# cristiano-nicolau/sudoku_solver_distributed

Measured on AMD Instinct MI355X. Metric: puzzles solved/sec (node), 1M hard 9x9 batch @1/2/4/8 GPU; single-puzzle p50 ms, higher is better.
Workload: dtype u8; 1 GPU; hard 17-clue 9x9 batch, 1048576 boards per step over all GPUs; global_batch=1048576, parallelism=shard1, steps_per_launch=32, inflight_per_gpu=2

## Files before the change

### sudoku_solver_distributed_amd/build.py

```python
from __future__ import annotations

import os
import subprocess
import sys

_HERE = os.path.dirname(os.path.abspath(__file__))
ROOT = os.path.dirname(_HERE)
_SCHED = os.environ.get("SDK_PLANE_SCHED", "iterative-ilp")


_LLVM_EXTRA = os.environ.get("SDK_PLANE_LLVM", "").split()


def sources(sched: str = _SCHED):
    extra = [f for o in _LLVM_EXTRA for f in ("-mllvm", o)]
    return (("sudoku_kernels.hip", []),
            ("plane_kernels.hip", ([] if sched == "default" else ["-mllvm", f"-amdgpu-sched-strategy={sched}"]) + extra),
            ("count_kernels.hip", ["-mllvm", "-amdgpu-sched-strategy=iterative-minreg"]),
            ("canon_kernels.hip", []),
            ("rate_kernels.hip", []),
            ("cand_kernels.hip", ["-mllvm", "-amdgpu-sched-strategy=iterative-minreg"]),
            ("min_kernels.hip", ["-mllvm", "-amdgpu-sched-strategy=iterative-minreg"]),
            ("sample_kernels.hip", ["-mllvm", "-amdgpu-sched-strategy=iterative-minreg"]),
            ("uniq_kernels.hip", ["-mllvm", "-amdgpu-sched-strategy=iterative-minreg"]),
            ("exact_kernels.hip", ["-mllvm", "-amdgpu-sched-strategy=iterative-minreg"]),
            ("enum_kernels.hip", ["-mllvm", "-amdgpu-sched-strategy=iterative-minreg"]),
            ("backdoor_kernels.hip", []),
            ("ua_kernels.hip", []),
            ("hit_kernels.hip", []))


SRCS = sources()
VARIANTS = {
    "default": ((), _SCHED),
    "stamps": (("SDK_PLANE_STAMPS=1",), _SCHED),
    "waves5": (("SDK_PLANE_WAVES_PER_EU=5",), _SCHED),
    "waves6": (("SDK_PLANE_WAVES_PER_EU=6",), _SCHED),
    "nopinacc": (("SDK_PLANE_PIN_ACC=0",), _SCHED),
    "sched-default": ((), "default"),
    "sched-minreg": ((), "iterative-minreg"),
    "sched-maxocc": ((), "iterative-maxocc"),
    "sched-max-ilp": ((), "max-ilp"),
}
OUT = os.path.join(_HERE, "libsudoku_hip.so")
ARCH = os.environ.get("SDK_OFFLOAD_ARCH", "gfx950")


def hipcc() -> str:
    for cand in (os.environ.get("HIPCC"), "/opt/rocm/bin/hipcc"):
        if cand and os.path.exists(cand):
            return cand
    return "hipcc"


def build(force: bool = False, verbose: bool = False, defines=(), out: str = OUT) -> str:
    csrc = os.path.join(_HERE, "csrc")
    deps = [os.path.join(csrc, f) for f in os.listdir(csrc) if not f.endswith(".o")] + [os.path.join(ROOT, "include", "sudoku_hip.h")]
    if (not force and os.path.exists(out)
            and all(os.path.getmtime(out) >= os.path.getmtime(d) for d in deps)):
        return out
    if tuple(defines) and tuple(defines) not in {v[0] for v in VARIANTS.values()}:
        sys.path.insert(0, os.path.join(ROOT, "scripts"))
        import store_hazard_check
        if store_hazard_check.check_build(SRCS, defines, "+".join(defines)):
            raise RuntimeError(f"wide-store data hazard in the build with {defines} (scripts/store_hazard_check.py)")
    objs = []
    for name, extra in SRCS:
        obj = out + "." + name + ".o"
        cmd = [hipcc(), f"--offload-arch={ARCH}", "-O3", "-std=c++17", "-fPIC", "-Wall", *extra,
               *[f"-D{d}" for d in defines],
               "-c", "-o", obj, os.path.join(csrc, name)]
        if verbose:
            cmd.append("-Rpass-analysis=kernel-resource-usage")
        subprocess.check_call(cmd)
        objs.append(obj)
    subprocess.check_call([hipcc(), f"--offload-arch={ARCH}", "-shared", "-fPIC", "-o", out + ".tmp", *objs])
    for obj in objs:
        os.remove(obj)
    os.replace(out + ".tmp", out)
    return out


if __name__ == "__main__":
    args = sys.argv[1:]
    defs = [a[2:] for a in args if a.startswith("-D")]
    tag = args[args.index("--tag") + 1] if "--tag" in args else None
    dst = os.path.join(_HERE, f"libsudoku_hip_{tag}.so") if tag else OUT
    print(build(force="--force" in args or bool(tag), verbose="-v" in args, defines=defs, out=dst))
```

### sudoku_solver_distributed_amd/csrc/common.h

```cpp
#ifndef SDK_COMMON_H
#define SDK_COMMON_H

#include <hip/hip_runtime.h>
#include <stdint.h>

#include <atomic>

#include "../../include/sudoku_hip.h"

#define WAVES_PER_BLOCK 4
#define SDK_DEFERRED 0x7FFF0001
#define BLOCK_THREADS (64 * WAVES_PER_BLOCK)

enum {
    WS_QUEUE = 0,
    WS_BEST = 1,
    WS_DEFER_COUNT = 2,
    WS_DEFER_OVER = 3,
    WS_ARM_WORDS = 4,
    WS_GEN = 4,
    WS_ERR_SLOT = 5,
    WS_STACK_BYTE = 256,
    WS_FINISHED = 8,
    WS_SOLVED = 9,
    WS_GUESSES = 10,
    WS_SWEEPS = 11,
    WS_DEFERRED = 12,
    WS_ASSIGNED = 13,
    WS_ERROR = 14,
    WS_RESERVED = 15,
    WS_WORDS = 16
};
#define SDK_ERR_POOL_WAIT 1u

__device__ __forceinline__ uint32_t lowbit(uint32_t x) { return x & (0u - x); }

__device__ __forceinline__ void wave_lds_sync()
{
    __builtin_amdgcn_fence(__ATOMIC_SEQ_CST, "wavefront");
    __builtin_amdgcn_s_waitcnt(0xC07F);
    __builtin_amdgcn_wave_barrier();
}

__device__ __forceinline__ bool wany(bool p) { return __builtin_amdgcn_ballot_w64(p) != 0; }

__device__ __forceinline__ uint32_t rdlane(uint32_t v, int l)
{
    return (uint32_t)__builtin_amdgcn_readlane((int)v, l);
}

__device__ __forceinline__ void cell_units(int cell, int &r, int &c, int &b)
{
    r = cell / 9;
    c = cell - r * 9;
    b = (r / 3) * 3 + c / 3;
}

__device__ __forceinline__ int order_cell(uint64_t eb0, uint64_t eb1, int order)
{
    if (order == SDK_ORDER_NODE)
        return eb0 ? __builtin_ctzll(eb0) : 64 + __builtin_ctzll(eb1);
    const int hi = eb1 ? 64 + 63 - __builtin_clzll(eb1) : 63 - __builtin_clzll(eb0);
    const int start = (hi / 9) * 9;
    if (start >= 64) return start + __builtin_ctzll(eb1 >> (start - 64));
    const uint64_t m = eb0 & (~0ull << start);
    return m ? __builtin_ctzll(m) : 64 + __builtin_ctzll(eb1);
}

template <typename K>
static inline int cached_occupancy(K kernel, int block, int fallback, int cap, std::atomic<int> &cache)
{
    int nb = cache.load();
    if (nb) return nb;
    if (hipOccupancyMaxActiveBlocksPerMultiprocessor(&nb, kernel, block, 0) != hipSuccess || nb <= 0) nb = fallback;
    if (nb > cap) nb = cap;
    cache.store(nb);
    return nb;
}

struct PlaneBatches {
    int64_t end[SDK_MAX_BATCHES];
    const uint8_t *in[SDK_MAX_BATCHES];
    uint8_t *out[SDK_MAX_BATCHES];
    int32_t *status[SDK_MAX_BATCHES];
    int count;
};
#define PLANE_BATCH_SHIFT 40
#define PLANE_LOCAL_MASK ((1ll << PLANE_BATCH_SHIFT) - 1)

hipError_t sdk_launch_plane(const uint8_t *puzzles, uint8_t *sols, int32_t *status, int64_t n,
                            unsigned long long *ws, uint32_t *stack, int64_t *defer_list, int ordered, int order,
                            int64_t threads, int pipelined, hipStream_t st);
hipError_t sdk_launch_plane_multi(const PlaneBatches &bs, unsigned long long *ws, uint32_t *stack,
                                  int64_t *defer_list, int order, int64_t threads, int pipelined, hipStream_t st);
int sdk_plane_blocks_per_cu();
#define PLANE_MAX_DEPTH 32
#ifndef SDK_PLANE_BLOCK
#define SDK_PLANE_BLOCK 64
#endif
#define PLANE_THREADS SDK_PLANE_BLOCK
#define PLANE_STACK_WORDS 32
#define PLANE_DEFER_CAP (1 << 20)
#define PLANE_POOL_XCDS 8
#define PLANE_POOL_CAP 16384
#define PLANE_POOL_REC 36
#define PLANE_POOL_CTL 32
#define PLANE_POOL_ARM_WORDS 4
#define PLANE_POOL_STRIDE (PLANE_POOL_CTL + PLANE_POOL_CAP * (PLANE_POOL_REC + 1))
#define PLANE_POOL_BYTES ((size_t)PLANE_POOL_XCDS * PLANE_POOL_STRIDE * 4)

#endif
```

### sudoku_solver_distributed_amd/csrc/plane_kernel.h

```cpp
#ifndef SDK_PLANE_KERNEL_H
#define SDK_PLANE_KERNEL_H

#include "plane_solver.h"
#include "plane_stack.h"
#include "plane_wide.h"

#ifndef SDK_PLANE_REFILL
#define SDK_PLANE_REFILL 3
#endif
#ifndef SDK_PLANE_TAIL
#define SDK_PLANE_TAIL 6
#endif
#ifndef SDK_PLANE_TAIL_MODE
#define SDK_PLANE_TAIL_MODE 1
#endif
#ifndef SDK_PLANE_PIPE_TAIL
#define SDK_PLANE_PIPE_TAIL 8
#endif
#ifndef SDK_PLANE_PIPE_TAIL_MODE
#define SDK_PLANE_PIPE_TAIL_MODE 1
#endif
#ifndef SDK_PLANE_CHUNK
#define SDK_PLANE_CHUNK 64
#endif
// ... 388 lines not shown
    wide::Stats ws_ = {0u, 0u, bguess};
    CancelHook hk = {best, pb};
    const int r = wide::solve(w, depth, stk, L, node_order, PLANE_MAX_DEPTH, ws_, hk, mst, mrv_after);
    st[2] += ws_.passes;
    st[1] += ws_.guesses;
    plane_wide_answer(r, w, pb, ws_.bguess, lane, L, io, ws, defer_list, best, st);
}

template <class IO>
__device__ __forceinline__ void plane_wide_tail(const uint32_t *recs, int k, int lane, __amdgpu_buffer_rsrc_t stack_rsrc,
                                             const IO &io, unsigned long long *__restrict__ ws,
                                             int64_t *__restrict__ defer_list, const int64_t *best, int node_order,
                                             uint32_t mrv_after, uint32_t (&st)[5])
{
    const wide::Lanes L = wide::lanes();
    for (int s = 0; s < k; ++s) {
        const uint32_t *rec = recs + PLANE_TAIL_REC * s;
        uint32_t w = rec[L.valid ? L.word : 0u];
        w = L.valid ? w : 0u;
        const int64_t pb = ((int64_t)__builtin_amdgcn_readfirstlane(rec[28]) << 32) |
                           (int64_t)(uint32_t)__builtin_amdgcn_readfirstlane(rec[27]);
        plane_wide_record(w, pb, __builtin_amdgcn_readfirstlane(rec[29]), __builtin_amdgcn_readfirstlane(rec[30]),
                          __builtin_amdgcn_readfirstlane(rec[31]), __builtin_amdgcn_readfirstlane(rec[32]), L, lane,
                          stack_rsrc, io, ws, defer_list, best, node_order, mrv_after, st);
    }
}

template <class IO>
__device__ __forceinline__ void plane_pool_drain(const PlanePool &pool, int lane, __amdgpu_buffer_rsrc_t stack_rsrc,
                                              const IO &io, unsigned long long *__restrict__ ws,
                                              int64_t *__restrict__ defer_list, const int64_t *best, int node_order,
                                              uint32_t mrv_after, uint32_t gen, uint32_t polls, uint32_t (&st)[5])
{
#if SDK_PLANE_STAMPS
    uint64_t d_ok = 0, d_fail = 0, d_poll = 0, c_claim = 0, c_wait = 0, c_solve = 0;
    uint64_t d_t = __builtin_amdgcn_s_memtime();
#endif
    const wide::Lanes L = wide::lanes();
    while (pool_load(pool.word(POOL_AVAIL)) > 0) {
        uint32_t h = 0;
        int32_t a = 0;
        if (lane == 0) {
            a = __hip_atomic_fetch_add(pool.word(POOL_AVAIL), -1, __ATOMIC_RELAXED, __HIP_MEMORY_SCOPE_AGENT);
            if (a > 0)
                h = __hip_atomic_fetch_add(pool.ctl + POOL_HEAD, 1u, __ATOMIC_RELAXED, __HIP_MEMORY_SCOPE_AGENT);
            else
                __hip_atomic_fetch_add(pool.word(POOL_AVAIL), 1, __ATOMIC_RELAXED, __HIP_MEMORY_SCOPE_AGENT);
        }
        if (__builtin_amdgcn_readfirstlane(a) <= 0) {
#if SDK_PLANE_STAMPS
            d_fail++;
#endif
            continue;
        }
        h = __builtin_amdgcn_readfirstlane(h);
#if SDK_PLANE_STAMPS
        d_ok++;
        {
            const uint64_t t1 = __builtin_amdgcn_s_memtime();
            c_claim += t1 - d_t;
            d_t = t1;
        }
#endif
        bool ready = false;
        for (uint32_t tries = 0; tries < polls; ++tries) {
            uint32_t f = 0;
            if (lane == 0) f = __hip_atomic_load(pool.flags + h, __ATOMIC_RELAXED, __HIP_MEMORY_SCOPE_AGENT);
            ready = __builtin_amdgcn_readfirstlane(f) == gen;
#if SDK_PLANE_STAMPS
            d_poll++;
#endif
            if (ready) break;
            __builtin_amdgcn_s_sleep(2);
        }
        if (!ready) {
            if (lane == 0) {
                atomicOr(&ws[WS_ERROR], (unsigned long long)SDK_ERR_POOL_WAIT);
                __hip_atomic_store(&ws[WS_ERR_SLOT], (unsigned long long)h, __ATOMIC_RELAXED, __HIP_MEMORY_SCOPE_AGENT);
            }
            break;
        }
#if SDK_PLANE_STAMPS
        {
            const uint64_t t1 = __builtin_amdgcn_s_memtime();
            c_wait += t1 - d_t;
            d_t = t1;
        }
#endif
#if SDK_PLANE_POOL_INV == 2
        __builtin_amdgcn_fence(__ATOMIC_ACQUIRE, "agent");
#elif SDK_PLANE_POOL_INV == 1
        asm volatile("buffer_inv sc0" ::: "memory");
#endif
        const uint32_t *rec = pool.recs + (size_t)h * PLANE_POOL_REC;
        const uint32_t rw = lane < 36 ? __hip_atomic_load(rec + lane, __ATOMIC_RELAXED, __HIP_MEMORY_SCOPE_AGENT) : 0u;
        uint32_t w = __builtin_amdgcn_ds_bpermute((int)(4u * (L.valid ? L.word : 0u)), (int)rw);
        w = L.valid ? w : 0u;
        const int64_t pb = ((int64_t)rdlane(rw, 28) << 32) | (int64_t)rdlane(rw, 27);
        plane_wide_record(w, pb, rdlane(rw, 29), rdlane(rw, 30), rdlane(rw, 31), rdlane(rw, 32), L, lane, stack_rsrc,
                          io, ws, defer_list, best, node_order, mrv_after, st);
#if SDK_PLANE_STAMPS
        {
            const uint64_t t1 = __builtin_amdgcn_s_memtime();
            c_solve += t1 - d_t;
            d_t = t1;
        }
#endif
    }
#if SDK_PLANE_STAMPS
    c_claim += __builtin_amdgcn_s_memtime() - d_t;
    if (lane == 0) {
        atomicAdd(&ws[24], (unsigned long long)d_ok);
        atomicAdd(&ws[25], (unsigned long long)d_fail);
        atomicAdd(&ws[26], (unsigned long long)d_poll);
        atomicAdd(&ws[27], (unsigned long long)c_claim);
        atomicAdd(&ws[28], (unsigned long long)c_wait);
        atomicAdd(&ws[29], (unsigned long long)c_solve);
    }
#endif
}

__device__ __forceinline__ uint32_t wave_sum(uint32_t v)
{
#pragma unroll
    for (int o = 32; o > 0; o >>= 1) v += (uint32_t)__shfl_xor((int)v, o);
    return v;
}

enum { PL_IDLE = 0, PL_ACTIVE = 1, PL_SOLVED = 2, PL_UNSOLVABLE = 3, PL_CANCELLED = 4 };

__device__ __forceinline__ unsigned long long rdlane64(unsigned long long v, int l)
{
    return ((unsigned long long)rdlane((uint32_t)(v >> 32), l) << 32) | rdlane((uint32_t)v, l);
}


#ifndef SDK_PLANE_WAVES_PER_EU
#define SDK_PLANE_WAVES_PER_EU 4
#endif
template <class IO>
__device__ __forceinline__ void plane_body(const IO &io, unsigned long long *__restrict__ ws,
                                           uint32_t *__restrict__ stack, int64_t *__restrict__ defer_list,
                                           int ordered, int order, int refill, int tail, int tail_mode, int chunk,
                                           uint32_t mrv_after, uint32_t pool_polls)
{
    const int64_t n = io.total();
    if (blockIdx.x == 0 && threadIdx.x == 0) atomicAdd(&ws[WS_ASSIGNED], (unsigned long long)n);
    __shared__ __attribute__((aligned(16))) uint32_t stage_lds[PLANE_THREADS / 64][PLANE_STAGE_DWORDS];
    __shared__ __attribute__((aligned(16))) uint32_t outbox_lds[PLANE_THREADS / 64][PLANE_OUTBOX * PLANE_OB_WORDS];
#if SDK_PLANE_LDS_PAD
    __shared__ uint32_t lds_pad[PLANE_THREADS / 64][SDK_PLANE_LDS_PAD];
    asm volatile("" ::"v"((uint32_t)(uintptr_t)&lds_pad[0][0]));
#endif
    uint32_t *stage = stage_lds[threadIdx.x >> 6];
    uint32_t *outbox = outbox_lds[threadIdx.x >> 6];
    uint32_t ob_count = 0;
    if ((threadIdx.x & 63) == 0) stage[PLANE_STAGE_DWORDS - 1] = 0u;
    const int64_t nt = (int64_t)gridDim.x * PLANE_THREADS;
    const int64_t g = (int64_t)blockIdx.x * PLANE_THREADS + threadIdx.x;
    PlaneStack stk = {
        __builtin_amdgcn_make_buffer_rsrc(stack, 0, (int)(nt * PLANE_MAX_DEPTH * 128), 0x00020000),
        (uint32_t)g * (uint32_t)(PLANE_MAX_DEPTH * 128)};
    const int64_t *best = ordered ? (const int64_t *)&ws[WS_BEST] : nullptr;
    const int node_order = order == SDK_ORDER_NODE;
    const int lane = threadIdx.x & 63;

    plane::Board B;
    int64_t p = -1;
    int state = PL_IDLE;
    uint32_t depth = 0;
    uint32_t fin = 0, solved = 0, guesses = 0, passes = 0, deferred = 0;
    uint32_t bguess = 0;
    uint32_t mst = 0;
    uint32_t und[3] = {0u, 0u, 0u}, nd[3] = {0u, 0u, 0u};
    bool drained = false;
    int64_t res_lo = 0, res_hi = 0;
    int64_t rec_base = 0;
    int64_t rec_id = 0;
    int64_t seg_hi = 0;
    bool queue_out = false;
    const int64_t nwaves = (int64_t)gridDim.x * (PLANE_THREADS / 64);
    uint64_t tail_act = 0;
#if SDK_PLANE_STAMPS
    const uint64_t st_t0 = __builtin_amdgcn_s_memrealtime();
    uint64_t st_t1 = 0;
    uint32_t st_after = 0, st_iters = 0;
    uint64_t st_piters = 0, st_lanes = 0, st_step = 0, st_push = 0, st_pop = 0;
    uint64_t st_pass = 0, st_io = 0, st_tail = 0, st_tb = 0;
    uint64_t st_atom = 0, st_dep = 0;
    uint64_t st_store = 0;
    uint64_t st_claims = 0;
#endif

    {
        const int64_t v0 = g - lane;
        queue_out = nt >= n;
        drained = queue_out;
        const int64_t kk = v0 < n ? (n - v0 < 64 ? n - v0 : 64) : 0;
        for (int64_t s0 = 0; s0 < kk;) {
            const int64_t sv = v0 + s0, cap = sv + PLANE_START_SPAN < v0 + kk ? sv + PLANE_START_SPAN : v0 + kk;
            const int64_t se = io.seg_end(sv, cap);
            const int cnt = (int)(se - sv);
            const uint32_t sh = plane_stage_span(io.seg_in(sv), io.seg_n(sv), io.seg_local(sv), cnt, stage, lane);
            const int r = lane - (int)s0;
            if (r >= 0 && r < cnt) {
                const int64_t q = io.id(sv) + r;
                uint32_t x[21];
                plane_stage_words(stage, sh + 81u * (uint32_t)r, x);
                bool clash;
                uint32_t given[3];
                const bool ok = plane::load_words(B, x, clash, given);
                const bool cancel = ok && best && __hip_atomic_load(best, __ATOMIC_RELAXED, __HIP_MEMORY_SCOPE_AGENT) < q;
                if (ok && !cancel) {
                    p = q;
                    depth = 0;
                    bguess = 0;
                    mst = 0;
#pragma unroll
                    for (int b = 0; b < 3; ++b) {
                        nd[b] = given[b];
                        und[b] = plane::andn(plane::ROWS, given[b]);
                    }
                    state = PL_ACTIVE;
                } else {
                    const uint8_t *src = io.src(q);
                    uint8_t *dst = io.dst(q);
                    for (int i = 0; i < 81; ++i) dst[i] = src[i];
                    *io.stat(q) = ok ? SDK_CANCELLED : SDK_INVALID;
                    fin++;
                }
            }
            s0 = se - v0;
            if (s0 < kk) wave_lds_sync();
        }
    }

    for (;;) {
#if SDK_PLANE_STAMPS
        const uint64_t st_ta = __builtin_amdgcn_s_memtime();
        if (st_tb) st_pass += st_ta - st_tb;
        st_iters++;
        if (drained) {
            if (!st_t1) st_t1 = __builtin_amdgcn_s_memrealtime();
            st_after++;
        }
#endif
        const uint64_t active = __builtin_amdgcn_ballot_w64(state == PL_ACTIVE);
        if (__builtin_popcountll(~active) >= refill || active == 0) {
            const int c0 = plane_slot_cell(lane, 0), c1 = plane_slot_cell(lane, 1);
#if SDK_PLANE_STAMPS
            const uint64_t st_s0 = __builtin_amdgcn_s_memtime();
#endif
            uint64_t m = __builtin_amdgcn_ballot_w64(state == PL_SOLVED);
#if !SDK_PLANE_ROOTFULL
            solved += state == PL_SOLVED;
            fin += state == PL_SOLVED;
#endif
            if (m) {
                const uint32_t ns = (uint32_t)__builtin_popcountll(m);
                if (ob_count + ns > (uint32_t)PLANE_OUTBOX) {
                    plane_flush_outbox(outbox, ob_count, lane, io, ws, defer_list, solved, fin, deferred);
                    ob_count = 0;
                }
                if (state == PL_SOLVED) {
                    sdk_v4u *rec = (sdk_v4u *)(outbox + PLANE_OB_WORDS * (ob_count + lanes_below(m)));
                    uint32_t V[4][3];
#pragma unroll
                    for (int b = 0; b < 3; ++b) {
                        V[0][b] = plane::or3(plane::or3(B.P[0][b], B.P[2][b], B.P[4][b]), B.P[6][b], B.P[8][b]);
                        V[1][b] = plane::or3(B.P[1][b], B.P[2][b], B.P[5][b] | B.P[6][b]);
                        V[2][b] = plane::or3(B.P[3][b], B.P[4][b], B.P[5][b] | B.P[6][b]);
                        V[3][b] = B.P[7][b] | B.P[8][b];
                    }
                    rec[0] = (sdk_v4u){V[0][0], V[0][1], V[0][2], V[1][0]};
                    rec[1] = (sdk_v4u){V[1][1], V[1][2], V[2][0], V[2][1]};
                    rec[2] = (sdk_v4u){V[2][2], V[3][0], V[3][1], V[3][2]};
                    rec[3] = (sdk_v4u){(uint32_t)p, (uint32_t)(p >> 32), 0u, 0u};
#if !SDK_PLANE_ROOTFULL
                    *io.stat(p) = SDK_SOLVED;
#endif
                }
                ob_count += ns;
            }
            m = __builtin_amdgcn_ballot_w64(state >= PL_UNSOLVABLE);
            while (m) {
                const int i = __builtin_ctzll(m);
                m &= m - 1;
                const int64_t pi = ((int64_t)rdlane((uint32_t)(p >> 32), i) << 32) | rdlane((uint32_t)p, i);
                const bool cancelled = rdlane((uint32_t)state, i) == PL_CANCELLED;
                if (!cancelled && plane_givens_clash(io.src(pi), c0, c1)) {
                    if (lane == i) {
                        plane_defer(io.stat(pi), pi, ws, defer_list);
                        deferred++;
                        guesses -= bguess;
                    }
                    continue;
                }
                plane_copy_board(io.src(pi), io.dst(pi), lane);
                if (lane == 0) {
                    *io.stat(pi) = cancelled ? SDK_CANCELLED : SDK_UNSOLVABLE;
                    fin++;
                }
            }
            if (state != PL_ACTIVE) state = PL_IDLE;
#if SDK_PLANE_STAMPS
            st_store += __builtin_amdgcn_s_memtime() - st_s0;
#endif
            if (!drained) {
                const uint64_t idle = ~active;
                const int k = __builtin_popcountll(idle);
                unsigned long long base = 0;
                const int leader = __builtin_ctzll(idle);
#if SDK_PLANE_STAMPS
                const uint64_t st_r0 = __builtin_amdgcn_s_memtime();
#endif
                if (res_lo == res_hi && !queue_out) {
                    const int64_t seen = res_hi > nt ? res_hi : nt;
                    int64_t c = chunk > 0 ? (n - seen) / (SDK_PLANE_GUIDE * nwaves) : 0;
                    c = c > chunk ? chunk : c;
                    c = c < k ? k : c;
                    c = c > PLANE_CHUNK_MAX ? PLANE_CHUNK_MAX : c;
                    if (lane == leader) base = atomicAdd(&ws[WS_QUEUE], (unsigned long long)c);
#if SDK_PLANE_STAMPS
                    st_claims = ((st_claims & 0xFFFFFFFFull) + 1) | ((uint64_t)c << 32);
#endif
                    base = __shfl(base, leader);
                    res_lo = nt + (int64_t)base;
                    res_hi = res_lo + c < n ? res_lo + c : n;
                    if (res_lo > n) res_lo = n;
                    queue_out = res_lo + c >= n;
                    if constexpr (!IO::multi) {
                        const int cc = __builtin_amdgcn_readfirstlane((int)(res_hi - res_lo));
                        rec_base = res_lo;
                        if (cc) {
                            const uint32_t sh = plane_stage_span(io.in, n, res_lo, cc, stage, lane);
                            plane_convert_chunk(stage, sh, cc, lane);
                        }
                    }
                    seg_hi = IO::multi ? res_lo : res_hi;
                }
                if (IO::multi && res_lo == seg_hi && res_lo < res_hi) {
                    seg_hi = io.seg_end(res_lo, res_hi);
                    const int cc = __builtin_amdgcn_readfirstlane((int)(seg_hi - res_lo));
                    rec_base = res_lo;
                    rec_id = io.id(res_lo);
                    const uint32_t sh = plane_stage_span(io.seg_in(res_lo), io.seg_n(res_lo), io.seg_local(res_lo), cc,
                                                         stage, lane);
                    plane_convert_chunk(stage, sh, cc, lane);
                }
                base = (unsigned long long)res_lo;
                const int64_t avail = (IO::multi ? seg_hi : res_hi) - res_lo;
                const int kk = __builtin_amdgcn_readfirstlane((int)(avail < k ? avail : k));
                res_lo += kk;
                drained = queue_out && res_lo == res_hi;
#if SDK_PLANE_STAMPS
                const uint64_t st_r1 = __builtin_amdgcn_s_memtime();
                st_atom += st_r1 - st_r0;
#endif
                if (kk) {
#if SDK_PLANE_STAMPS
                    const uint64_t st_r2 = __builtin_amdgcn_s_memtime();
#endif
                    const uint32_t rank = lanes_below(idle);
                    const bool take = ((idle >> lane) & 1u) && rank < (uint32_t)kk;
                    const uint64_t loaded = __builtin_amdgcn_ballot_w64(take);
                    bool bad = false;
                    if (take) {
                        const uint32_t *rec = stage + PLANE_REC * ((uint32_t)(base - (unsigned long long)rec_base) + rank);
                        uint32_t V[4][3], given[3];
#pragma unroll
                        for (int s = 0; s < 4; ++s)
#pragma unroll
                            for (int b = 0; b < 3; ++b) V[s][b] = rec[3 * s + b];
                        bad = rec[12] != 0u;
                        p = (IO::multi ? rec_id + ((int64_t)base - rec_base) : (int64_t)base) + (int64_t)rank;
                        depth = 0;
                        bguess = 0;
                        mst = 0;
                        if (!bad && !(best && __hip_atomic_load(best, __ATOMIC_RELAXED, __HIP_MEMORY_SCOPE_AGENT) < p)) {
                            plane::planes_from_slices(B, V, given);
#pragma unroll
                            for (int b = 0; b < 3; ++b) {
                                nd[b] = given[b];
                                und[b] = plane::andn(plane::ROWS, given[b]);
                            }
                            state = PL_ACTIVE;
                        } else {
                            state = PL_CANCELLED;
                        }
                    }
                    const uint64_t badm = __builtin_amdgcn_ballot_w64(bad);
                    uint64_t r = loaded & __builtin_amdgcn_ballot_w64(state != PL_ACTIVE);
                    while (r) {
                        const int i = __builtin_ctzll(r);
                        r &= r - 1;
                        const int64_t q = (IO::multi ? rec_id + ((int64_t)base - rec_base) : (int64_t)base) +
                                          (int64_t)__builtin_popcountll(loaded & ((1ull << i) - 1));
                        plane_copy_board(io.src(q), io.dst(q), lane);
                        if (lane == 0) {
                            *io.stat(q) = ((badm >> i) & 1u) ? SDK_INVALID : SDK_CANCELLED;
                            fin++;
                        }
                    }
                    if (state == PL_CANCELLED) state = PL_IDLE;
#if SDK_PLANE_STAMPS
                    st_dep += __builtin_amdgcn_s_memtime() - st_r2;
#endif
                }
            }
            if (drained && tail > 0) {
                const uint64_t act = __builtin_amdgcn_ballot_w64(state == PL_ACTIVE);
                if (act && __builtin_popcountll(act) <= tail) {
                    tail_act = act;
                    break;
                }
            }
            if (drained && __builtin_amdgcn_ballot_w64(state != PL_IDLE) == 0) break;
        }
#if SDK_PLANE_STAMPS
        st_tb = __builtin_amdgcn_s_memtime();
        st_io += st_tb - st_ta;
#endif
        if (state != PL_ACTIVE) continue;

        passes++;
#if SDK_PLANE_STAMPS
        st_lanes += (uint32_t)__builtin_popcountll(__builtin_amdgcn_ballot_w64(true));
        st_piters++;
#endif
        const int r = plane::pass_ahead(B, und, nd);
        if (r == plane::STUCK && best && __hip_atomic_load(best, __ATOMIC_RELAXED, __HIP_MEMORY_SCOPE_AGENT) < p) {
            state = PL_CANCELLED;
            continue;
        }
        const uint32_t gb = bguess;
#if SDK_PLANE_STAMPS
        const uint32_t st_d0 = depth;
        const uint64_t st_s0 = __builtin_amdgcn_s_memtime();
#endif
        const int s = plane::search_step_ahead(B, und, nd, r, depth, mst, stk, node_order, PLANE_MAX_DEPTH, mrv_after,
                                               bguess, SDK_PLANE_ROOTFULL && best == nullptr);
#if SDK_PLANE_STAMPS
        st_step += __builtin_amdgcn_s_memtime() - st_s0;
        st_push += wany(bguess != gb) ? 1u : 0u;
        st_pop += wany(depth < st_d0) ? 1u : 0u;
#endif
        guesses += bguess - gb;
        if (s == plane::S_SOLVED) {
            state = PL_SOLVED;
            if (best)
                __hip_atomic_fetch_min((int64_t *)&ws[WS_BEST], p, __ATOMIC_RELAXED, __HIP_MEMORY_SCOPE_AGENT);
        } else if (s == plane::S_NONE) {
            state = PL_UNSOLVABLE;
        } else if (s == plane::S_DEEP) {
            plane_defer(io.stat(p), p, ws, defer_list);
            deferred++;
            guesses -= bguess;
            state = PL_IDLE;
        }
    }
    if (ob_count) plane_flush_outbox(outbox, ob_count, lane, io, ws, defer_list, solved, fin, deferred);
#if SDK_PLANE_STAMPS
    const uint64_t st_tt = __builtin_amdgcn_s_memtime();
    const uint64_t st_t3 = __builtin_amdgcn_s_memrealtime();
    const uint32_t st_tailn = (uint32_t)__builtin_popcountll(tail_act);
    uint32_t st_tailp = 0;
#endif
    const PlanePool pool = plane_pool(defer_list);
    const uint32_t gen = tail_mode >= 2 ? __builtin_amdgcn_readfirstlane((uint32_t)ws[WS_GEN]) : 0u;
    if (tail_act) {
        __builtin_amdgcn_s_waitcnt(SDK_WAIT_VM0);
        const uint32_t k = (uint32_t)__builtin_popcountll(tail_act);
        const uint32_t rank = lanes_below(tail_act);
        uint32_t fit = 0, slot0 = 0;
        if (tail_mode >= 2) {
            slot0 = (uint32_t)pool_add(pool.word(POOL_RESERVED), (int32_t)k);
            fit = slot0 >= PLANE_POOL_CAP ? 0u : (PLANE_POOL_CAP - slot0 < k ? PLANE_POOL_CAP - slot0 : k);
        }
        if ((tail_act >> lane) & 1u) {
            uint32_t v[PLANE_POOL_REC];
#pragma unroll
            for (int w = 0; w < 27; ++w) v[w] = B.P[w / 3][w % 3];
            v[27] = (uint32_t)p;
            v[28] = (uint32_t)(p >> 32);
            v[29] = depth;
            v[30] = stk.lane_off;
            v[31] = bguess;
            v[32] = mst;
            v[33] = v[34] = v[35] = 0u;
            if (rank < fit) {
                sdk_v4u *q = (sdk_v4u *)(pool.recs + (size_t)(slot0 + rank) * PLANE_POOL_REC);
#pragma unroll
                for (int i = 0; i < PLANE_POOL_REC / 4; ++i)
                    q[i] = sdk_v4u{v[4 * i], v[4 * i + 1], v[4 * i + 2], v[4 * i + 3]};
            } else {
                uint32_t *rec = stage + PLANE_TAIL_REC * (rank - fit);
#pragma unroll
                for (int w = 0; w < PLANE_TAIL_REC; ++w) rec[w] = v[w];
            }
        }
        if (fit) pool_publish(pool, slot0, fit, gen, lane);
        wave_lds_sync();
        uint32_t wst[5] = {0u, 0u, 0u, 0u, 0u};
        if (k > fit)
            plane_wide_tail(stage, (int)(k - fit), lane, stk.rsrc, io, ws, defer_list, best, node_order, mrv_after,
                            wst);
#if SDK_PLANE_STAMPS
        st_tailp = wst[2];
#endif
        if (lane == 0) {
            solved += wst[0];
            guesses += wst[1];
            passes += wst[2];
            fin += wst[4];
            deferred += wst[3];
        }
    }
    if (tail_mode >= 2) {
        uint32_t wst[5] = {0u, 0u, 0u, 0u, 0u};
        plane_pool_drain(pool, lane, stk.rsrc, io, ws, defer_list, best, node_order, mrv_after, gen, pool_polls, wst);
        if (lane == 0) {
            solved += wst[0];
            guesses += wst[1];
            passes += wst[2];
            fin += wst[4];
            deferred += wst[3];
        }
    }
#if SDK_PLANE_STAMPS
    {
        st_tail = __builtin_amdgcn_s_memtime() - st_tt;
        int64_t *st = defer_list + (PLANE_DEFER_CAP / 2) + 32 * (g >> 6);
        const uint64_t t2 = __builtin_amdgcn_s_memrealtime();
        if (lane == 0) st[0] = (int64_t)st_t0;
        if (lane == 1) st[1] = (int64_t)(st_t1 ? st_t1 : t2);
        if (lane == 2) st[2] = (int64_t)t2;
        if (lane == 3) st[3] = (int64_t)st_after;
        if (lane == 4) st[4] = (int64_t)st_pass;
        if (lane == 5) st[5] = (int64_t)st_io;
        if (lane == 6) st[6] = (int64_t)st_tail;
        if (lane == 7) st[7] = (int64_t)st_iters;
        if (lane == 8) st[8] = (int64_t)st_atom;
        if (lane == 9) st[9] = 0;
        if (lane == 10) st[10] = (int64_t)st_dep;
        if (lane == 11) st[11] = (int64_t)st_store;
        if (lane == 12) st[12] = (int64_t)st_t3;
        if (lane == 13) st[13] = (int64_t)st_tailn;
        if (lane == 14) st[14] = (int64_t)st_tailp;
        if (lane == 15) st[15] = (int64_t)st_claims;
        if (lane == 16) st[16] = (int64_t)st_piters;
        if (lane == 17) st[17] = (int64_t)st_lanes;
        if (lane == 18) st[18] = (int64_t)st_step;
        if (lane == 19) st[19] = (int64_t)st_push;
        if (lane == 20) st[20] = (int64_t)st_pop;
    }
#endif
    fin = wave_sum(fin);
    solved = wave_sum(solved);
    guesses = wave_sum(guesses);
    passes = wave_sum(passes);
    deferred = wave_sum(deferred);
    if (lane == 0 && deferred) atomicAdd(&ws[WS_DEFERRED], (unsigned long long)deferred);
    if (lane == 0 && (fin | deferred | passes)) {
        atomicAdd(&ws[WS_FINISHED], (unsigned long long)(long long)(int32_t)fin);
        atomicAdd(&ws[WS_SOLVED], (unsigned long long)solved);
        atomicAdd(&ws[WS_GUESSES], (unsigned long long)(long long)(int32_t)guesses);
        atomicAdd(&ws[WS_SWEEPS], (unsigned long long)passes);
    }
}

__global__ __launch_bounds__(PLANE_THREADS, SDK_PLANE_WAVES_PER_EU) void plane_kernel(
    const uint8_t *__restrict__ puzzles, uint8_t *__restrict__ sols, int32_t *__restrict__ status, int64_t n,
    unsigned long long *__restrict__ ws, uint32_t *__restrict__ stack, int64_t *__restrict__ defer_list, int ordered,
    int order, int refill, int tail, int tail_mode, int chunk, uint32_t mrv_after, uint32_t pool_polls)
{
    const PlaneIO1 io = {puzzles, sols, status, n};
    plane_body(io, ws, stack, defer_list, ordered, order, refill, tail, tail_mode, chunk, mrv_after, pool_polls);
}

__global__ __launch_bounds__(PLANE_THREADS, SDK_PLANE_WAVES_PER_EU) void plane_kernel_multi(
    const PlaneBatches bs, unsigned long long *__restrict__ ws, uint32_t *__restrict__ stack,
    int64_t *__restrict__ defer_list, int order, int refill, int tail, int tail_mode, int chunk, uint32_t mrv_after,
    uint32_t pool_polls)
// ... 7 lines not shown
```

### sudoku_solver_distributed_amd/csrc/plane_solver.h

```cpp
#ifndef SDK_PLANE_SOLVER_H
#define SDK_PLANE_SOLVER_H

#include <stdint.h>

#ifdef __HIPCC__
#define PS_FN __host__ __device__ __forceinline__
#define PS_MF __host__ __device__ __forceinline__
#else
#define PS_FN static inline
#define PS_MF inline
#endif

#if defined(__HIPCC__) && defined(__HIP_DEVICE_COMPILE__)
#define PS_PIN(x) asm volatile("" : "+v"(x))
#else
#define PS_PIN(x) ((void)0)
#endif
#ifndef SDK_PLANE_PIN_ACC
#define SDK_PLANE_PIN_ACC 1
#endif
#ifndef SDK_PLANE_LC
#define SDK_PLANE_LC 3
#endif
#ifndef SDK_WIDE_LC
#define SDK_WIDE_LC SDK_PLANE_LC
#endif
#ifndef SDK_PLANE_GROUP
#define SDK_PLANE_GROUP 1
#endif
#ifndef SDK_PLANE_HX
#define SDK_PLANE_HX 1
#endif
#if SDK_PLANE_HX && !(SDK_PLANE_LC & 1)
#undef SDK_PLANE_HX
#define SDK_PLANE_HX 0
#endif

namespace plane {

enum : uint32_t {
    ROWS = 0x1FFu | (0x1FFu << 10) | (0x1FFu << 20),
    GUARDS = (1u << 9) | (1u << 19) | (1u << 29),
    ONES = 1u | (1u << 10) | (1u << 20),
    KDEC = GUARDS - ONES,
    BOXC = 0x49u,
};

enum { OPEN = 0, DEAD = 1, SOLVED = 2, STUCK = 3 };

struct Board {
    uint32_t P[9][3];
    uint32_t Det[3];
};

PS_FN void pin_board(Board &B)
{
#pragma unroll
    for (int d = 0; d < 9; ++d)
#pragma unroll
        for (int b = 0; b < 3; ++b) PS_PIN(B.P[d][b]);
}

PS_FN constexpr int cell_band(int i) { return i / 27; }
PS_FN constexpr int cell_pos(int i) { return 10 * ((i / 9) % 3) + i % 9; }
PS_FN int pos_cell(int b, int pos) { return 27 * b + 9 * (pos / 10) + pos % 10; }

#if defined(__HIPCC__) && defined(__HIP_DEVICE_COMPILE__)
template <uint32_t K>
__device__ __forceinline__ uint32_t vconst()
{
    uint32_t r;
    asm("v_mov_b32 %0, %1" : "=v"(r) : "i"(K));
    return r;
}
template <unsigned TT>
__device__ __forceinline__ uint32_t bop3(uint32_t a, uint32_t b, uint32_t c)
{
    return __builtin_amdgcn_bitop3_b32(a, b, c, TT);
}
#define PS_BOP3(TT, a, b, c, host) bop3<TT>(a, b, c)
#else
#define PS_BOP3(TT, a, b, c, host) (host)
#endif
PS_FN uint32_t or3(uint32_t a, uint32_t b, uint32_t c) { return PS_BOP3(0xFE, a, b, c, a | b | c); }
PS_FN uint32_t maj3(uint32_t a, uint32_t b, uint32_t c) { return PS_BOP3(0xE8, a, b, c, (a & b) | (c & (a | b))); }
PS_FN uint32_t xor3(uint32_t a, uint32_t b, uint32_t c) { return PS_BOP3(0x96, a, b, c, a ^ b ^ c); }
PS_FN uint32_t andn(uint32_t a, uint32_t b) { return PS_BOP3(0x30, a, b, b, a & ~b); }
PS_FN uint32_t andn2(uint32_t a, uint32_t b, uint32_t c) { return PS_BOP3(0x10, a, b, c, a & ~b & ~c); }
PS_FN uint32_t and_andn(uint32_t a, uint32_t b, uint32_t c) { return PS_BOP3(0x40, a, b, c, a & b & ~c); }
PS_FN uint32_t or_and(uint32_t a, uint32_t b, uint32_t c) { return PS_BOP3(0xF8, a, b, c, a | (b & c)); }
PS_FN uint32_t or_andn(uint32_t a, uint32_t b, uint32_t c) { return PS_BOP3(0xF4, a, b, c, a | (b & ~c)); }
PS_FN uint32_t and3(uint32_t a, uint32_t b, uint32_t c) { return PS_BOP3(0x80, a, b, c, a & b & c); }
PS_FN uint32_t andn_and(uint32_t a, uint32_t b, uint32_t c) { return PS_BOP3(0x70, a, b, c, a & ~(b & c)); }
PS_FN uint32_t sel(uint32_t m, uint32_t a, uint32_t b) { return PS_BOP3(0xCA, m, a, b, (m & a) | (~m & b)); }
PS_FN uint32_t bop3_nor(uint32_t a, uint32_t b, uint32_t c) { return PS_BOP3(0xEF, a, b, c, ~a | b | c); }
PS_FN uint32_t mul24(uint32_t c, uint32_t k) { return (c & 0xFFFFFFu) * k; }
#ifndef SDK_PLANE_MUL16
#define SDK_PLANE_MUL16 1
#endif
PS_FN uint32_t box_one(uint32_t x, uint32_t m)
{
#if defined(__HIPCC__) && defined(__HIP_DEVICE_COMPILE__)
    return bop3<0x20>(x, m, vconst<BOXC>());
#else
    return x & ~m & BOXC;
#endif
}
PS_FN uint32_t box_cols(uint32_t c)
{
#if SDK_PLANE_MUL16 && defined(__HIPCC__) && defined(__HIP_DEVICE_COMPILE__)
    uint32_t r = c;
    asm("v_mul_lo_u16 %0, 7, %0" : "+v"(r));
    return r;
#else
    return mul24(c, 7u);
#endif
}

PS_FN void point_rows_parts(uint32_t y, uint32_t &rows, uint32_t &area)
{
    const uint32_t r3 = or3(y, y >> 1, y >> 2) & 0x4912449u;
    const uint32_t a1 = r3 >> 10, a2 = r3 >> 20;
    const uint32_t hbox = box_one(xor3(r3, a1, a2), maj3(r3, a1, a2));
    area = mul24(hbox, 0x701C07u);
    const uint32_t rn = ((r3 & area) + ROWS) & GUARDS;
    rows = rn - (rn >> 9);
}
PS_FN uint32_t point_rows(uint32_t y)
{
    uint32_t rows, area;
    point_rows_parts(y, rows, area);
    return andn(rows, area);
}
PS_FN uint32_t point_rows_apply(uint32_t y)
{
    uint32_t rows, area;
    point_rows_parts(y, rows, area);
    return PS_BOP3(0xB0, y, rows, area, y & ~(rows & ~area));
}

PS_FN uint32_t spread_rows(uint32_t c) { return c | (c << 10) | (c << 20); }
PS_FN uint32_t guard_rows(uint32_t g) { return g - (g >> 9); }
PS_FN uint32_t row_nonzero(uint32_t y) { return (y + ROWS) & GUARDS; }
PS_FN uint32_t fold_rows(uint32_t y) { return (y | (y >> 10) | (y >> 20)) & 0x1FFu; }

struct Board;
PS_FN void pin_board(Board &B);

PS_FN uint32_t rule_a(const Board &B, uint32_t (&single)[3])
{
    uint32_t empty = 0;
#pragma unroll
    for (int b = 0; b < 3; ++b) {
        uint32_t o = B.P[0][b] | B.P[1][b];
        const uint32_t m23 = maj3(o, B.P[2][b], B.P[3][b]);
        o = or3(o, B.P[2][b], B.P[3][b]);
        const uint32_t m45 = maj3(o, B.P[4][b], B.P[5][b]);
        o = or3(o, B.P[4][b], B.P[5][b]);
        uint32_t t = or_and(m23, B.P[0][b], B.P[1][b]);
        t = or3(t, m45, maj3(o, B.P[6][b], B.P[7][b]));
        o = or3(o, B.P[6][b], B.P[7][b]);
        t = or_and(t, o, B.P[8][b]);
        o |= B.P[8][b];
        empty = or_andn(empty, ROWS, o);
        single[b] = andn(o, t);
    }
    return empty;
}

PS_FN uint32_t pass_body(Board &B, const uint32_t (&nd)[3], uint32_t (&hall)[3])
{
    hall[0] = hall[1] = hall[2] = 0u;
#if SDK_PLANE_GROUP > 1
    uint32_t hgrp[3] = {0u, 0u, 0u};
#endif
    uint32_t rowall = GUARDS, colall = 0x1FFu, boxall = BOXC;
#pragma unroll
    for (int d = 0; d < 9; ++d) {
        uint32_t x[3], f[3];
#pragma unroll
        for (int b = 0; b < 3; ++b) {
#if SDK_PLANE_GROUP > 1
            if (d >= SDK_PLANE_GROUP) B.P[d][b] = andn(B.P[d][b], hgrp[b]);
#else
            if (d > 0) B.P[d][b] = andn(B.P[d][b], hall[b]);
#endif
            x[b] = nd[b] & B.P[d][b];
            f[b] = or3(x[b], x[b] >> 10, x[b] >> 20);
        }
        const uint32_t cpeer = mul24(or3(f[0], f[1], f[2]) & 0x1FFu, 0x100401u);
#pragma unroll
        for (int b = 0; b < 3; ++b) {
            const uint32_t g = or3(f[b], f[b] >> 1, f[b] >> 2);
            const uint32_t rn = (x[b] + ROWS) & GUARDS;
            const uint32_t peer = or3(rn - (rn >> 9), cpeer, mul24(g & BOXC, 0x701C07u));
            B.P[d][b] = sel(peer, x[b], B.P[d][b]);
        }
        uint32_t o[3], t[3], gr[3], hb[3];
#if SDK_PLANE_LC
        uint32_t vp[3];
#endif
#pragma unroll
        for (int b = 0; b < 3; ++b) {
            const uint32_t y = B.P[d][b];
            const uint32_t y1 = y + ROWS;
            rowall &= y1;
            const uint32_t z = y & y1;
            const uint32_t nz = (z + ROWS) & GUARDS;
            gr[b] = nz - (nz >> 9);
            const uint32_t s1 = y >> 10, s2 = y >> 20;
            o[b] = or3(y, s1, s2);
            t[b] = maj3(y, s1, s2);
            const uint32_t o1 = o[b] >> 1, o2 = o[b] >> 2;
            const uint32_t ob = or3(o[b], o1, o2);
            boxall &= ob;
            const uint32_t mo = maj3(o[b], o1, o2);
#if SDK_PLANE_HX
            const uint32_t vb = box_one(xor3(o[b], o1, o2), mo);
            vp[b] = o[b] & box_cols(vb);
            hb[b] = andn(vp[b], t[b]);
#else
            const uint32_t tb = or3(t[b], t[b] >> 1, t[b] >> 2);
            const uint32_t q = andn2(ob, tb, mo) & BOXC;
            hb[b] = mul24(q, 0x701C07u);
#if SDK_PLANE_LC
            const uint32_t vb = andn(xor3(o[b], o1, o2), mo) & BOXC;
            vp[b] = o[b] & box_cols(vb);
#endif
#endif
        }
        const uint32_t O = or3(o[0], o[1], o[2]);
        colall &= O;
        const uint32_t mo3 = maj3(o[0], o[1], o[2]);
        const uint32_t hc = andn2(O, or3(t[0], t[1], t[2]), mo3) & 0x1FFu;
#if SDK_PLANE_HX
#pragma unroll
        for (int b = 0; b < 3; ++b) hb[b] = mul24(hb[b] | hc, 0x100401u);
        const uint32_t hcol = 0u;
#else
        const uint32_t hcol = mul24(hc, 0x100401u);
#endif
#if SDK_PLANE_LC
        {
            const uint32_t vpa = or3(vp[0], vp[1], vp[2]);
            const uint32_t one_band = andn(xor3(o[0], o[1], o[2]), mo3) & 0x1FFu;
            (void)vpa;
            (void)one_band;
#pragma unroll
            for (int b = 0; b < 3; ++b) {
                uint32_t ec = 0;
#if SDK_PLANE_LC & 1
                ec = andn(vpa, vp[b]);
#endif
#if SDK_PLANE_LC & 4
                {
                    const uint32_t cc = o[b] & one_band;
                    ec |= andn(mul24(or3(cc, cc >> 1, cc >> 2) & BOXC, 7u), cc);
                }
#endif
                const uint32_t e = mul24(ec, 0x100401u);
                B.P[d][b] = andn(B.P[d][b], e);
            }
        }
#endif
#pragma unroll
        for (int b = 0; b < 3; ++b) {
            const uint32_t hs = bop3_nor(gr[b], hb[b], hcol);
#if SDK_PLANE_GROUP > 1
            if (d % SDK_PLANE_GROUP) {
                const uint32_t p = B.P[d][b];
                B.P[d][b] = PS_BOP3(0xB0, p, hall[b], hs, p & ~(hall[b] & ~hs));
                hall[b] = or_and(hall[b], p, hs);
                continue;
            }
#endif
            hall[b] = or_and(hall[b], B.P[d][b], hs);
        }
#if SDK_PLANE_GROUP > 1
        if (d % SDK_PLANE_GROUP != SDK_PLANE_GROUP - 1 && d != 8) continue;
#pragma unroll
        for (int b = 0; b < 3; ++b) hgrp[b] = hall[b];
#endif
        pin_board(B);
#if SDK_PLANE_PIN_ACC
        PS_PIN(rowall);
        PS_PIN(colall);
        PS_PIN(boxall);
#pragma unroll
        for (int b = 0; b < 3; ++b) PS_PIN(hall[b]);
#endif
    }
#pragma unroll
    for (int b = 0; b < 3; ++b) {
        uint32_t later = B.P[8][b];
#pragma unroll
        for (int e = 7; e >= 0; --e) {
            B.P[e][b] = andn_and(B.P[e][b], hall[b], later);
            if (e) later |= B.P[e][b];
        }
    }
#if SDK_PLANE_LC & 2
    {
#pragma unroll
        for (int d = 0; d < 9; ++d)
#pragma unroll
            for (int b = 0; b < 3; ++b) {
                B.P[d][b] = point_rows_apply(B.P[d][b]);
                PS_PIN(B.P[d][b]);
            }
    }
#endif
    return or3(rowall ^ GUARDS, colall ^ 0x1FFu, (boxall & BOXC) ^ BOXC);
}

PS_FN int pass(Board &B, uint32_t und[3])
{
    uint32_t single[3], nd[3], hall[3];
    uint32_t dead = rule_a(B, single);
#pragma unroll
    for (int b = 0; b < 3; ++b) {
        nd[b] = andn(single[b], B.Det[b]);
        B.Det[b] = single[b];
        und[b] = andn(ROWS, single[b]);
    }
    const bool all_single = and3(single[0], single[1], single[2]) == ROWS;
    const bool any_nd = or3(nd[0], nd[1], nd[2]) != 0;
    pin_board(B);
    dead |= pass_body(B, nd, hall);
    if (dead) return DEAD;
    if (all_single) return SOLVED;
    const bool newh = or3(hall[0] & und[0], hall[1] & und[1], hall[2] & und[2]) != 0;
    return (any_nd || newh) ? OPEN : STUCK;
}

PS_FN int pass_ahead(Board &B, uint32_t (&und)[3], uint32_t (&nd)[3])
{
    uint32_t single[3], hall[3];
    const bool all_single = or3(und[0], und[1], und[2]) == 0;
    pin_board(B);
    uint32_t dead = pass_body(B, nd, hall);
    const bool newh = or3(hall[0] & und[0], hall[1] & und[1], hall[2] & und[2]) != 0;
    dead |= rule_a(B, single);
#pragma unroll
    for (int b = 0; b < 3; ++b) {
        nd[b] = single[b] & und[b];
        und[b] = andn(ROWS, single[b]);
    }
    if (dead) return DEAD;
    if (all_single) return SOLVED;
    const bool any_nd = or3(nd[0], nd[1], nd[2]) != 0;
    return (any_nd || newh) ? OPEN : STUCK;
}

PS_FN void pick_cell(const uint32_t und[3], int node_order, int &band, int &pos)
{
    if (node_order) {
        band = und[0] ? 0 : und[1] ? 1 : 2;
        const uint32_t w = band == 0 ? und[0] : band == 1 ? und[1] : und[2];
        pos = __builtin_ctz(w);
    } else {
        band = und[2] ? 2 : und[1] ? 1 : 0;
        const uint32_t w = band == 0 ? und[0] : band == 1 ? und[1] : und[2];
        const int hi = 31 - __builtin_clz(w);
        const int k = hi >= 20 ? 2 : hi >= 10 ? 1 : 0;
        pos = 10 * k + __builtin_ctz(w >> (10 * k));
    }
}

#ifndef SDK_PLANE_MRV_PICK
#define SDK_PLANE_MRV_PICK 0
#endif
PS_FN void pick_mrv_masks(const uint32_t (&e2)[3], const uint32_t (&e3)[3], const uint32_t und[3], int &band,
                          int &pos)
{
#if SDK_PLANE_MRV_PICK
    uint32_t r[9];
#pragma unroll
    for (int b = 0; b < 3; ++b) {
        r[3 * b] = e2[b] & 0x1FFu;
        r[3 * b + 1] = (e2[b] >> 10) & 0x1FFu;
        r[3 * b + 2] = e2[b] >> 20;
    }
    const uint32_t sa = xor3(r[0], r[1], r[2]), ca = maj3(r[0], r[1], r[2]);
    const uint32_t sb = xor3(r[3], r[4], r[5]), cb = maj3(r[3], r[4], r[5]);
    const uint32_t sc = xor3(r[6], r[7], r[8]), cc = maj3(r[6], r[7], r[8]);
    const uint32_t c1 = xor3(sa, sb, sc), cd = maj3(sa, sb, sc);
    const uint32_t se = xor3(ca, cb, cc), ce = maj3(ca, cb, cc);
    const uint32_t c2 = se ^ cd, cf = se & cd;
    const uint32_t c4 = ce ^ cf, c8 = ce & cf;
    uint32_t m = or3(c1, c2, c4 | c8);
    uint32_t t = m & c8;
    m = t ? t : m;
    t = m & c4;
    m = t ? t : m;
    t = m & c2;
    m = t ? t : m;
    t = m & c1;
    m = t ? t : m;
    if (m) {
        const uint32_t col = spread_rows(m & (0u - m));
        band = (e2[0] & col) ? 0 : (e2[1] & col) ? 1 : 2;
        pos = __builtin_ctz((band == 0 ? e2[0] : band == 1 ? e2[1] : e2[2]) & col);
        return;
    }
#endif
    const uint32_t w[3] = {e2[0] ? e2[0] : e3[0] ? e3[0] : und[0], e2[1] ? e2[1] : e3[1] ? e3[1] : und[1],
                           e2[2] ? e2[2] : e3[2] ? e3[2] : und[2]};
    const int k2 = e2[0] ? 0 : e2[1] ? 1 : e2[2] ? 2 : -1;
    const int k3 = e3[0] ? 0 : e3[1] ? 1 : e3[2] ? 2 : -1;
    band = k2 >= 0 ? k2 : k3 >= 0 ? k3 : (und[0] ? 0 : und[1] ? 1 : 2);
    pos = __builtin_ctz(band == 0 ? w[0] : band == 1 ? w[1] : w[2]);
}

#ifndef SDK_PLANE_COUNT_PICK
#define SDK_PLANE_COUNT_PICK pick_count_masks
#endif
PS_FN void pick_count_masks(const uint32_t (&e2)[3], const uint32_t (&e3)[3], const uint32_t und[3], int &band,
                            int &pos)
{
    const bool a2 = or3(e2[0], e2[1], e2[2]) != 0, a3 = or3(e3[0], e3[1], e3[2]) != 0;
    uint32_t s[3], key[3];
#pragma unroll
    for (int b = 0; b < 3; ++b) {
        s[b] = a2 ? e2[b] : a3 ? e3[b] : und[b];
        key[b] = ((uint32_t)__builtin_popcount(s[b]) - 1u) * 32u + (27u - (uint32_t)__builtin_popcount(und[b]));
    }
    band = key[1] < key[0] ? 1 : 0;
    const uint32_t k01 = key[1] < key[0] ? key[1] : key[0];
    band = key[2] < k01 ? 2 : band;
    pos = __builtin_ctz(band == 0 ? s[0] : band == 1 ? s[1] : s[2]);
}

PS_FN void cand_masks(const Board &B, const uint32_t und[3], uint32_t (&e2)[3], uint32_t (&e3)[3])
{
#pragma unroll
    for (int b = 0; b < 3; ++b) {
        const uint32_t *p = &B.P[0][b];
#define PL(d) p[3 * (d)]
        const uint32_t sa = xor3(PL(0), PL(1), PL(2)), ca = maj3(PL(0), PL(1), PL(2));
        const uint32_t sb = xor3(PL(3), PL(4), PL(5)), cb = maj3(PL(3), PL(4), PL(5));
        const uint32_t sc = xor3(PL(6), PL(7), PL(8)), cc = maj3(PL(6), PL(7), PL(8));
#undef PL
        const uint32_t s0 = xor3(sa, sb, sc), cd = maj3(sa, sb, sc);
        const uint32_t se = xor3(ca, cb, cc), ce = maj3(ca, cb, cc);
        const uint32_t s1 = se ^ cd, cf = se & cd;
        const uint32_t hi = ce | cf;
        e2[b] = and_andn(und[b], s1, s0 | hi);
        e3[b] = and3(und[b], s1, s0) & ~hi;
    }
}

PS_FN void pick_mrv(const Board &B, const uint32_t und[3], int &band, int &pos)
{
    uint32_t e2[3], e3[3];
    cand_masks(B, und, e2, e3);
    pick_mrv_masks(e2, e3, und, band, pos);
}

PS_FN void pick_count(const Board &B, const uint32_t und[3], int &band, int &pos)
{
    uint32_t e2[3], e3[3];
    cand_masks(B, und, e2, e3);
    SDK_PLANE_COUNT_PICK(e2, e3, und, band, pos);
}

PS_FN uint32_t band_word(const uint32_t (&w)[3], int band) { return band == 0 ? w[0] : band == 1 ? w[1] : w[2]; }

PS_FN uint32_t cell_cand(const Board &B, int band, int pos)
{
    const uint32_t cb = 1u << pos;
    const uint32_t m0 = band == 0 ? cb : 0u, m1 = band == 1 ? cb : 0u, m2 = band == 2 ? cb : 0u;
    uint32_t c = 0;
#pragma unroll
    for (int d = 8; d >= 0; --d) {
        const uint32_t x = or_and(or_and(B.P[d][0] & m0, B.P[d][1], m1), B.P[d][2], m2);
        c = c + c + (x >> pos);
    }
    return c;
}

PS_FN void set_cell(Board &B, int band, int pos, uint32_t dbit)
{
    const uint32_t cb = 1u << pos;
    const uint32_t m[3] = {band == 0 ? cb : 0u, band == 1 ? cb : 0u, band == 2 ? cb : 0u};
#pragma unroll
    for (int d = 0; d < 9; ++d) {
        const uint32_t other = ((dbit >> d) & 1u) - 1u;
#pragma unroll
        for (int b = 0; b < 3; ++b) B.P[d][b] = andn_and(B.P[d][b], m[b], other);
    }
}

PS_FN void planes_from_slices(Board &B, const uint32_t (&V)[4][3], uint32_t (&given)[3])
{
#pragma unroll
    for (int b = 0; b < 3; ++b) {
        const uint32_t v0 = V[0][b], v1 = V[1][b], v2 = V[2][b], v3 = V[3][b];
        const uint32_t lo[4] = {andn2(ROWS, v0, v1), andn(v0, v1), andn(v1, v0), v0 & v1};
        const uint32_t hi[3] = {andn2(ROWS, v2, v3), andn(v2, v3), andn(v3, v2)};
        const uint32_t e = lo[0] & hi[0];
        given[b] = andn(ROWS, e);
#pragma unroll
        for (int d = 0; d < 9; ++d) {
            const int v = d + 1;
// ... 409 lines not shown
```

Baseline: 1.468 billion boards/s.

## Replace pointing-rows bit logic with LDS lookup table in plane solver

Adds a 512-entry LDS table, filled per block at kernel start, that maps a 9-bit box-occupancy signature of each digit-band plane to a keep-mask for the pointing (locked candidates) elimination. Each of the 27 plane/band words now gets a computed byte offset, one LDS read and an AND, replacing the ALU-heavy point_rows_apply sequence. To amortise the table fill and allow sharing, the default plane block size grows from 64 to 256 threads, and the wave index becomes uniform via readfirstlane. The trade is LDS latency, possible bank conflicts and a block-wide sync against fewer VALU ops, with possible occupancy changes from the larger block.

New measurement: 1.599 billion boards/s, median of 6. 1.09x the previous value.

```diff
diff --git a/sudoku_solver_distributed_amd/build.py b/sudoku_solver_distributed_amd/build.py
--- a/sudoku_solver_distributed_amd/build.py
+++ b/sudoku_solver_distributed_amd/build.py
@@ -37,6 +37,7 @@
     "waves5": (("SDK_PLANE_WAVES_PER_EU=5",), _SCHED),
     "waves6": (("SDK_PLANE_WAVES_PER_EU=6",), _SCHED),
     "nopinacc": (("SDK_PLANE_PIN_ACC=0",), _SCHED),
+    "locktbl-off": (("SDK_PLANE_LOCKTBL=0",), _SCHED),
     "sched-default": ((), "default"),
     "sched-minreg": ((), "iterative-minreg"),
     "sched-maxocc": ((), "iterative-maxocc"),
diff --git a/sudoku_solver_distributed_amd/csrc/common.h b/sudoku_solver_distributed_amd/csrc/common.h
--- a/sudoku_solver_distributed_amd/csrc/common.h
+++ b/sudoku_solver_distributed_amd/csrc/common.h
@@ -95,8 +95,11 @@
                                   int64_t *defer_list, int order, int64_t threads, int pipelined, hipStream_t st);
 int sdk_plane_blocks_per_cu();
 #define PLANE_MAX_DEPTH 32
+#ifndef SDK_PLANE_LOCKTBL
+#define SDK_PLANE_LOCKTBL 1
+#endif
 #ifndef SDK_PLANE_BLOCK
-#define SDK_PLANE_BLOCK 64
+#define SDK_PLANE_BLOCK (SDK_PLANE_LOCKTBL ? 256 : 64)
 #endif
 #define PLANE_THREADS SDK_PLANE_BLOCK
 #define PLANE_STACK_WORDS 32
diff --git a/sudoku_solver_distributed_amd/csrc/plane_kernel.h b/sudoku_solver_distributed_amd/csrc/plane_kernel.h
--- a/sudoku_solver_distributed_amd/csrc/plane_kernel.h
+++ b/sudoku_solver_distributed_amd/csrc/plane_kernel.h
@@ -564,8 +564,14 @@
     __shared__ uint32_t lds_pad[PLANE_THREADS / 64][SDK_PLANE_LDS_PAD];
     asm volatile("" ::"v"((uint32_t)(uintptr_t)&lds_pad[0][0]));
 #endif
-    uint32_t *stage = stage_lds[threadIdx.x >> 6];
-    uint32_t *outbox = outbox_lds[threadIdx.x >> 6];
+#if SDK_PLANE_LOCKTBL
+    __shared__ uint32_t lock_lds[plane::LOCK_ENTRIES];
+    plane::lock_fill(lock_lds, threadIdx.x, PLANE_THREADS);
+    __syncthreads();
+#endif
+    const uint32_t wv = PLANE_THREADS > 64 ? (uint32_t)__builtin_amdgcn_readfirstlane((int)(threadIdx.x >> 6)) : threadIdx.x >> 6;
+    uint32_t *stage = stage_lds[wv];
+    uint32_t *outbox = outbox_lds[wv];
     uint32_t ob_count = 0;
     if ((threadIdx.x & 63) == 0) stage[PLANE_STAGE_DWORDS - 1] = 0u;
     const int64_t nt = (int64_t)gridDim.x * PLANE_THREADS;
@@ -840,7 +846,11 @@
         st_lanes += (uint32_t)__builtin_popcountll(__builtin_amdgcn_ballot_w64(true));
         st_piters++;
 #endif
+#if SDK_PLANE_LOCKTBL
+        const int r = plane::pass_ahead(B, und, nd, lock_lds);
+#else
         const int r = plane::pass_ahead(B, und, nd);
+#endif
         if (r == plane::STUCK && best && __hip_atomic_load(best, __ATOMIC_RELAXED, __HIP_MEMORY_SCOPE_AGENT) < p) {
             state = PL_CANCELLED;
             continue;
diff --git a/sudoku_solver_distributed_amd/csrc/plane_solver.h b/sudoku_solver_distributed_amd/csrc/plane_solver.h
--- a/sudoku_solver_distributed_amd/csrc/plane_solver.h
+++ b/sudoku_solver_distributed_amd/csrc/plane_solver.h
@@ -139,6 +139,44 @@
     return PS_BOP3(0xB0, y, rows, area, y & ~(rows & ~area));
 }
 
+enum { LOCK_ENTRIES = 512 };
+#ifndef SDK_PLANE_LOCKTBL_GROUP
+#define SDK_PLANE_LOCKTBL_GROUP 9
+#endif
+PS_FN uint32_t twice(uint32_t x)
+{
+#if defined(__HIPCC__) && defined(__HIP_DEVICE_COMPILE__)
+    uint32_t r;
+    asm("v_add_u32 %0, %1, %1" : "=v"(r) : "v"(x));
+    return r;
+#else
+    return x + x;
+#endif
+}
+PS_FN uint32_t lock_offset(uint32_t y)
+{
+    const uint32_t y2 = twice(y), y4 = twice(y2);
+    const uint32_t r3 = or3(y, y2, y4) & (0x4912449u << 2);
+    return or3(r3, r3 >> 9, r3 >> 18) & 0x7FCu;
+}
+PS_FN uint32_t lock_index(uint32_t y) { return lock_offset(y) >> 2; }
+PS_FN uint32_t lock_entry(uint32_t i)
+{
+    uint32_t rep = 0;
+    for (int j = 0; j < 3; ++j)
+        for (int k = 0; k < 3; ++k)
+            if ((i >> (3 * j + k)) & 1u) rep |= 7u << (10 * k + 3 * j);
+    return ROWS & ~point_rows(rep);
+}
+PS_FN void lock_fill(uint32_t *tbl, uint32_t tid, uint32_t nthreads)
+{
+    for (uint32_t i = tid; i < (uint32_t)LOCK_ENTRIES; i += nthreads) tbl[i] = lock_entry(i);
+}
+PS_FN uint32_t lock_read(const uint32_t *tbl, uint32_t off)
+{
+    return *(const uint32_t *)((const unsigned char *)tbl + off);
+}
+
 PS_FN uint32_t spread_rows(uint32_t c) { return c | (c << 10) | (c << 20); }
 PS_FN uint32_t guard_rows(uint32_t g) { return g - (g >> 9); }
 PS_FN uint32_t row_nonzero(uint32_t y) { return (y + ROWS) & GUARDS; }
@@ -168,7 +206,8 @@
     return empty;
 }
 
-PS_FN uint32_t pass_body(Board &B, const uint32_t (&nd)[3], uint32_t (&hall)[3])
+template <bool TBL>
+PS_FN uint32_t pass_body_t(Board &B, const uint32_t (&nd)[3], uint32_t (&hall)[3], const uint32_t *tbl)
 {
     hall[0] = hall[1] = hall[2] = 0u;
 #if SDK_PLANE_GROUP > 1
@@ -300,7 +339,27 @@
         }
     }
 #if SDK_PLANE_LC & 2
-    {
+    if constexpr (TBL) {
+        constexpr int G = SDK_PLANE_LOCKTBL_GROUP;
+        static_assert(G >= 1 && 27 % G == 0, "SDK_PLANE_LOCKTBL_GROUP divides 27");
+#pragma unroll
+        for (int g = 0; g < 27; g += G) {
+            uint32_t off[G], keep[G];
+#pragma unroll
+            for (int i = 0; i < G; ++i) off[i] = lock_offset(B.P[(g + i) / 3][(g + i) % 3]);
+#pragma unroll
+            for (int i = 0; i < G; ++i) PS_PIN(off[i]);
+#pragma unroll
+            for (int i = 0; i < G; ++i) keep[i] = lock_read(tbl, off[i]);
+#pragma unroll
+            for (int i = 0; i < G; ++i) PS_PIN(keep[i]);
+#pragma unroll
+            for (int i = 0; i < G; ++i) {
+                B.P[(g + i) / 3][(g + i) % 3] &= keep[i];
+                PS_PIN(B.P[(g + i) / 3][(g + i) % 3]);
+            }
+        }
+    } else {
 #pragma unroll
         for (int d = 0; d < 9; ++d)
 #pragma unroll
@@ -310,10 +369,20 @@
             }
     }
 #endif
+    (void)tbl;
     return or3(rowall ^ GUARDS, colall ^ 0x1FFu, (boxall & BOXC) ^ BOXC);
 }
-
-PS_FN int pass(Board &B, uint32_t und[3])
+PS_FN uint32_t pass_body(Board &B, const uint32_t (&nd)[3], uint32_t (&hall)[3])
+{
+    return pass_body_t<false>(B, nd, hall, nullptr);
+}
+PS_FN uint32_t pass_body(Board &B, const uint32_t (&nd)[3], uint32_t (&hall)[3], const uint32_t *tbl)
+{
+    return pass_body_t<true>(B, nd, hall, tbl);
+}
+
+template <bool TBL>
+PS_FN int pass_t(Board &B, uint32_t und[3], const uint32_t *tbl)
 {
     uint32_t single[3], nd[3], hall[3];
     uint32_t dead = rule_a(B, single);
@@ -326,19 +395,22 @@
     const bool all_single = and3(single[0], single[1], single[2]) == ROWS;
     const bool any_nd = or3(nd[0], nd[1], nd[2]) != 0;
     pin_board(B);
-    dead |= pass_body(B, nd, hall);
+    dead |= pass_body_t<TBL>(B, nd, hall, tbl);
     if (dead) return DEAD;
     if (all_single) return SOLVED;
     const bool newh = or3(hall[0] & und[0], hall[1] & und[1], hall[2] & und[2]) != 0;
     return (any_nd || newh) ? OPEN : STUCK;
 }
-
-PS_FN int pass_ahead(Board &B, uint32_t (&und)[3], uint32_t (&nd)[3])
+PS_FN int pass(Board &B, uint32_t und[3]) { return pass_t<false>(B, und, nullptr); }
+PS_FN int pass(Board &B, uint32_t und[3], const uint32_t *tbl) { return pass_t<true>(B, und, tbl); }
+
+template <bool TBL>
+PS_FN int pass_ahead_t(Board &B, uint32_t (&und)[3], uint32_t (&nd)[3], const uint32_t *tbl)
 {
     uint32_t single[3], hall[3];
     const bool all_single = or3(und[0], und[1], und[2]) == 0;
     pin_board(B);
-    uint32_t dead = pass_body(B, nd, hall);
+    uint32_t dead = pass_body_t<TBL>(B, nd, hall, tbl);
     const bool newh = or3(hall[0] & und[0], hall[1] & und[1], hall[2] & und[2]) != 0;
     dead |= rule_a(B, single);
 #pragma unroll
@@ -350,6 +422,14 @@
     if (all_single) return SOLVED;
     const bool any_nd = or3(nd[0], nd[1], nd[2]) != 0;
     return (any_nd || newh) ? OPEN : STUCK;
+}
+PS_FN int pass_ahead(Board &B, uint32_t (&und)[3], uint32_t (&nd)[3])
+{
+    return pass_ahead_t<false>(B, und, nd, nullptr);
+}
+PS_FN int pass_ahead(Board &B, uint32_t (&und)[3], uint32_t (&nd)[3], const uint32_t *tbl)
+{
+    return pass_ahead_t<true>(B, und, nd, tbl);
 }
 
 PS_FN void pick_cell(const uint32_t und[3], int node_order, int &band, int &pos)
```
